# microsoft/DFOL-VQA

Measured on AMD Instinct MI355X. Metric: questions/sec (GQA programs, N=100 objects), higher is better.
Workload: dtype f32

## Files before the change

### dfol_vqa_amd/csrc/dfol_pair_h2.hip

```cpp
#include "dfol_common.h"

#include <stdlib.h>

#include <type_traits>

#ifdef DFOL_PAIR_TRACE
__device__ long long dfol_h2_trace_buf[8 * 8 * 64];
#define TRACE(slot)                                                                                                  \
    do {                                                                                                             \
        if (trace_on && lane == 0) dfol_h2_trace_buf[(trace_blk * 8 + wave) * 64 + (slot)] = clock64();              \
    } while (0)
#else
#define TRACE(slot)
#endif

#ifndef DFOL_H2_PREFETCH
#define DFOL_H2_PREFETCH 1
#endif
#ifndef DFOL_H2_BDEPTH
#define DFOL_H2_BDEPTH 2
#endif
#ifndef DFOL_H2_DMA_ASM
#define DFOL_H2_DMA_ASM 1
#endif
#ifndef DFOL_H2T_SKIP
#define DFOL_H2T_SKIP 0
#endif
#ifndef DFOL_H2_DMA_LATE
#define DFOL_H2_DMA_LATE 0
#endif


namespace {

typedef float floatx4 __attribute__((ext_vector_type(4)));
typedef _Float16 f16x8 __attribute__((ext_vector_type(8)));
typedef _Float16 f16x2 __attribute__((ext_vector_type(2)));
typedef float f32x2 __attribute__((ext_vector_type(2)));
typedef uint32_t u32x4 __attribute__((ext_vector_type(4)));

constexpr float H2_NL2E = -1.44269504088896340736f;
constexpr int H2_CH = 32;
constexpr int H2_ROWS = 320, H2_TILES = 20;
constexpr int H2_PIECES = 2 * H2_ROWS * 4;
constexpr float H2_AMAX = 60000.0f;
constexpr float H2_L2E = 1.44269504088896340736f;
constexpr float H2_LN2 = 0.69314718055994530942f;

__device__ __forceinline__ int h2_swz(int row) { return (4 - ((row >> 2) & 3)) & 3; }

__device__ __forceinline__ void h2_split2(float x0, float x1, uint32_t& h, uint32_t& l) {
    const f32x2 x = {x0, x1};
    const f16x2 hh = __builtin_convertvector(x, f16x2);
    const f32x2 r = x - __builtin_convertvector(hh, f32x2);
    const f16x2 ll = __builtin_convertvector(r, f16x2);
    h = __builtin_bit_cast(uint32_t, hh);
    l = __builtin_bit_cast(uint32_t, ll);
}

__device__ __forceinline__ float h2_elu_neg(float zs) {
    const float p = __builtin_amdgcn_fmed3f(__builtin_amdgcn_exp2f(zs), 0.0f, 1.0f);
    return fmaf(p, H2_L2E, -H2_L2E);
}

__host__ __device__ __forceinline__ constexpr int h2_kperm(int kq, int e) { return 16 * (e >> 2) + 4 * kq + (e & 3); }

template <bool HI>
__device__ __forceinline__ float h2_resid(float x, uint32_t hpair) {
    float r;
    if (HI) asm("v_fma_mix_f32 %0, -%1, 1.0, %2 op_sel:[1,0,0] op_sel_hi:[1,0,0]" : "=v"(r) : "v"(hpair), "v"(x));
    else asm("v_fma_mix_f32 %0, -%1, 1.0, %2 op_sel:[0,0,0] op_sel_hi:[1,0,0]" : "=v"(r) : "v"(hpair), "v"(x));
    return r;
}

__global__ void h2_row_scale_kernel(const float* __restrict__ W2, int64_t ld_w2, int HID2, int HID1, float* __restrict__ tail) {
    const int lane = threadIdx.x & 63, r = blockIdx.x * (blockDim.x >> 6) + (threadIdx.x >> 6);
    if (r >= H2_ROWS) return;
    float m = 0.f;
    if (r < HID2)
        for (int k = lane; k < HID1; k += 64) m = fmaxf(m, fabsf(W2[(int64_t)r * ld_w2 + k] * H2_LN2));
#pragma unroll
    for (int s = 32; s >= 1; s >>= 1) m = fmaxf(m, __shfl_xor(m, s, 64));
    int e = 0;
    if (m > 0.f && m < 3.0e38f) {
        int x;
        (void)frexpf(m, &x);
        e = 14 - x;
        e = e < -100 ? -100 : (e > 100 ? 100 : e);
    }
    if (lane == 0) {
        tail[r] = ldexpf(H2_NL2E, -e);
        reinterpret_cast<int32_t*>(tail)[H2_ROWS + r] = e;
    }
}

__global__ void h2_pack_w2_kernel(const float* __restrict__ W2, int64_t ld_w2, int HID2, int HID1, const float* __restrict__ tail,
                                  u32x4* __restrict__ out) {
    const int idx = blockIdx.x * blockDim.x + threadIdx.x;
    if (idx >= (HID1 / H2_CH) * H2_PIECES) return;
    const int c = idx / H2_PIECES, rem = idx - c * H2_PIECES;
    const int p = rem / (H2_ROWS * 4), rr = rem - p * H2_ROWS * 4, r = rr >> 2, slot = rr & 3;
    const int kq = slot ^ h2_swz(r);
    const int e = reinterpret_cast<const int32_t*>(tail)[H2_ROWS + r];
    uint32_t piece[4];
#pragma unroll
    for (int j = 0; j < 4; ++j) {
        float w0 = 0.f, w1 = 0.f;
        if (r < HID2) {
            w0 = ldexpf(W2[(int64_t)r * ld_w2 + c * H2_CH + h2_kperm(kq, 2 * j)] * H2_LN2, e);
            w1 = ldexpf(W2[(int64_t)r * ld_w2 + c * H2_CH + h2_kperm(kq, 2 * j + 1)] * H2_LN2, e);
        }
        uint32_t h, l;
        h2_split2(w0, w1, h, l);
        piece[j] = p == 0 ? h : l;
    }
    out[idx] = u32x4{piece[0], piece[1], piece[2], piece[3]};
}

struct H2Train {
    float* Z;
    float* pre2;
    int64_t ld_pre2;
    float* geo;
    float* x;
    int64_t ld_x;
    const int64_t* pair_off;
};

template <int NB16, bool TBF16, bool TRAIN = false>
__global__ __launch_bounds__(512) __attribute__((amdgpu_waves_per_eu(2, 2))) void pair_ll32h_kernel(
    const float* UV , int64_t ld_uv, int HID1, const float* __restrict__ pos, int64_t ld_pos,
    const float* __restrict__ Wg, const u32x4* __restrict__ W2h, const float* __restrict__ b2, int HID2,
    const float* __restrict__ E, int64_t ld_e, const float* __restrict__ be, const int32_t* __restrict__ n_obj,
    const int32_t* __restrict__ obj_off, int Q, int tiles_per_image, const int32_t* __restrict__ req_col,
    const int32_t* __restrict__ req_tile, const uint8_t* __restrict__ req_orient, int K, int NS, float dflt,
    void* __restrict__ tiles_v, H2Train tr) {
    constexpr int MT = 2, WAVES = 8;
    constexpr int ROWS = NB16 * 16, T = WAVES * 64, SLOTS = MT * 16 * WAVES;
    static_assert(NB16 > 16 && NB16 <= H2_TILES, "geometry");
    __shared__ __attribute__((aligned(16))) u32x4 Bs[2 * H2_PIECES];
    __shared__ __attribute__((aligned(16))) u32x4 WgA[(256 / H2_CH) * 2 * 64];
    constexpr int STAGE_FLOATS = 8192;
    __shared__ __attribute__((aligned(16))) float stage[STAGE_FLOATS];
    const int q = blockIdx.x / tiles_per_image, tb = blockIdx.x - q * tiles_per_image;
    const int n = n_obj[q], npairs = n * (n - 1);
    if (tb * SLOTS >= npairs) return;
    bool any = TRAIN;
    for (int k = 0; k < K; ++k) any |= req_col[(int64_t)k * Q + q] >= 0;
    if (!any) return;
    const int64_t prow0 = TRAIN ? tr.pair_off[q] : 0;

    const int tid = threadIdx.x, lane = tid & 63, wave = __builtin_amdgcn_readfirstlane(tid >> 6), kh = lane >> 4, r16 = lane & 15;
#ifdef DFOL_PAIR_TRACE
    const int trace_blk = ((int)blockIdx.x - 3000) / 500;
    const bool trace_on = blockIdx.x >= 3000 && (blockIdx.x - 3000) % 500 == 0 && trace_blk < 8;
#endif
    TRACE(0);
    const int nchunk = HID1 / H2_CH, lastc = nchunk - 1;
#pragma unroll
    for (int i = 0; i < H2_PIECES / T; ++i)
        __builtin_amdgcn_global_load_lds(W2h + T * i + tid, (__attribute__((address_space(3))) void*)&Bs[T * i + wave * 64], 16, 0, 0);
    const float* cf = reinterpret_cast<const float*>(W2h + (int64_t)nchunk * H2_PIECES);
    const int first = obj_off[q];
    u32x4 geoB[MT];
    const char* img_uv = reinterpret_cast<const char*>(UV + (int64_t)first * ld_uv);
    uint32_t uoff[MT], voff[MT];
    uint32_t zoff[MT];
#pragma unroll
    for (int m = 0; m < MT; ++m) {
        const int e_slot = tb * SLOTS + wave * (MT * 16) + m * 16 + r16;
        const bool valid = e_slot < npairs;
        zoff[m] = (TRAIN && valid) ? (uint32_t)(e_slot * HID1 + 4 * kh) * 4u : 0xffffffffu;
        const int s = valid ? e_slot / (n - 1) : 0, oo_ = valid ? e_slot - s * (n - 1) : 0, o = oo_ + (oo_ >= s);
        const float* ps = pos + (int64_t)(first + s) * ld_pos;
        const float* po = pos + (int64_t)(first + o) * ld_pos;
        const float x1 = ps[0], y1 = ps[1], w1 = ps[2], h1 = ps[3], x2 = po[0], y2 = po[1], w2 = po[2], h2 = po[3];
        const float dx = x1 + w1 / 2.0f - x2 - w2 / 2.0f, dy = y1 + h1 / 2.0f - y2 - h2 / 2.0f;
        const float dist = sqrtf(dx * dx + dy * dy);
        uint32_t gh01, gl01, gh23, gl23;
        const float ang = asinf(dy / fmaxf(dist, 1e-10f));
        const float sgx = (x2 - x1 > 0.f) ? 1.f : ((x2 - x1 < 0.f) ? -1.f : 0.f), sgy = (y2 - y1 > 0.f) ? 1.f : ((y2 - y1 < 0.f) ? -1.f : 0.f);
        h2_split2(dist, ang, gh01, gl01);
        h2_split2(sgx, sgy, gh23, gl23);
        if (TRAIN && valid && kh == 0) *reinterpret_cast<floatx4*>(tr.geo + (prow0 + e_slot) * 4) = floatx4{dist, ang, sgx, sgy};
        geoB[m] = kh == 0 ? u32x4{gh01, gh23, gl01, gl23} : (kh == 1 ? u32x4{gh01, gh23, 0u, 0u} : u32x4{0u, 0u, 0u, 0u});
        uoff[m] = (uint32_t)(s * (int)ld_uv + 4 * kh) * 4u;
        voff[m] = (uint32_t)(o * (int)ld_uv + HID1 + 4 * kh) * 4u;
    }
    for (int i = tid; i < (HID1 / 16) * 64; i += T) {
        const int kt = i >> 6, ln = i & 63, khh = ln >> 4;
        u32x4 frag = {0u, 0u, 0u, 0u};
        if (khh < 2) {
            const float4 g = *reinterpret_cast<const float4*>(Wg + (kt * 16 + (ln & 15)) * 4);
            uint32_t h01, l01, h23, l23;
            h2_split2(g.x * H2_L2E, g.y * H2_L2E, h01, l01);
            h2_split2(g.z * H2_L2E, g.w * H2_L2E, h23, l23);
            frag = khh == 0 ? u32x4{h01, h23, h01, h23} : u32x4{l01, l23, 0u, 0u};
        }
        WgA[i] = frag;
    }
    constexpr int SR = STAGE_FLOATS / ROWS - 2;
    for (int i = tid; i < ROWS; i += T) {
        stage[i] = H2_NL2E * (i < HID2 ? b2[i] : -1.0e30f);
        stage[ROWS + i] = i < HID2 ? cf[i] : 0.f;
    }
    const int Kc = K < SR ? K : SR;
    for (int k = 0; k < Kc; ++k) {
        const int col = req_col[(int64_t)k * Q + q];
        for (int i = tid; i < ROWS; i += T) stage[ROWS * (2 + k) + i] = (col >= 0 && i < HID2) ? E[(int64_t)col * ld_e + i] : 0.f;
    }

    floatx4 acc[MT][NB16];
#pragma unroll
    for (int m = 0; m < MT; ++m)
#pragma unroll
        for (int i = 0; i < NB16; ++i) acc[m][i] = floatx4{0.f, 0.f, 0.f, 0.f};

    auto dma_chunk = [&](int c, int buf) __attribute__((always_inline)) {
        const int w = wave - 4;
        constexpr int PER_WAVE = H2_PIECES / 4;
        const u32x4* src = W2h + (int64_t)c * H2_PIECES + w * PER_WAVE + lane;
        u32x4* dst = &Bs[buf * H2_PIECES + w * PER_WAVE];
#pragma unroll
        for (int g = 0; g < PER_WAVE / 64; g += 4) {
#if DFOL_H2_DMA_ASM
            const uint32_t d = (uint32_t)(uintptr_t)(__attribute__((address_space(3))) void*)(dst + 64 * g);
            const u32x4* sp = src + 64 * g;
#pragma clang diagnostic push
#pragma clang diagnostic ignored "-Winline-asm"
            const uint32_t m0v = __builtin_amdgcn_readfirstlane(d);
            const int rem = PER_WAVE / 64 - g;
            if (rem >= 4)
                asm volatile("s_mov_b32 m0, %1\n\ts_nop 0\n\tglobal_load_lds_dwordx4 %0, off\n\tglobal_load_lds_dwordx4 %0, off offset:1024\n\t"
                             "global_load_lds_dwordx4 %0, off offset:2048\n\tglobal_load_lds_dwordx4 %0, off offset:3072" ::"v"(sp), "s"(m0v) : "memory", "m0");
            else if (rem == 3)
                asm volatile("s_mov_b32 m0, %1\n\ts_nop 0\n\tglobal_load_lds_dwordx4 %0, off\n\tglobal_load_lds_dwordx4 %0, off offset:1024\n\t"
                             "global_load_lds_dwordx4 %0, off offset:2048" ::"v"(sp), "s"(m0v) : "memory", "m0");
            else if (rem == 2)
                asm volatile("s_mov_b32 m0, %1\n\ts_nop 0\n\tglobal_load_lds_dwordx4 %0, off\n\tglobal_load_lds_dwordx4 %0, off offset:1024" ::"v"(sp), "s"(m0v) : "memory", "m0");
            else
                asm volatile("s_mov_b32 m0, %1\n\ts_nop 0\n\tglobal_load_lds_dwordx4 %0, off" ::"v"(sp), "s"(m0v) : "memory", "m0");
#pragma clang diagnostic pop
#else
            auto d = (__attribute__((address_space(3))) void*)(dst + 64 * g);
            __builtin_amdgcn_global_load_lds(src + 64 * g, d, 16, 0, 0);
            if (g + 1 < PER_WAVE / 64) __builtin_amdgcn_global_load_lds(src + 64 * g, d, 16, 1024, 0);
            if (g + 2 < PER_WAVE / 64) __builtin_amdgcn_global_load_lds(src + 64 * g, d, 16, 2048, 0);
            if (g + 3 < PER_WAVE / 64) __builtin_amdgcn_global_load_lds(src + 64 * g, d, 16, 3072, 0);
#endif
        }
    };
    floatx4 ru[MT][2], rv[MT][2];
    auto load_uv = [&](int c) __attribute__((always_inline)) {
        const char* base = img_uv + (uint32_t)__builtin_amdgcn_readfirstlane(H2_CH * 4 * c);
#pragma unroll
        for (int m = 0; m < MT; ++m)
#pragma unroll
            for (int half = 0; half < 2; ++half) {
                ru[m][half] = *reinterpret_cast<const floatx4*>(base + uoff[m] + 64 * half);
                rv[m][half] = *reinterpret_cast<const floatx4*>(base + voff[m] + 64 * half);
            }
    };
    u32x4 ap[MT][2];
    auto make_a = [&](int c) __attribute__((always_inline)) {
        floatx4 z[MT][2];
#pragma unroll
        for (int t = 0; t < 2; ++t) {
            const f16x8 wa = __builtin_bit_cast(f16x8, WgA[(2 * c + t) * 64 + lane]);
#pragma unroll
            for (int m = 0; m < MT; ++m)
                z[m][t] = __builtin_amdgcn_mfma_f32_16x16x32_f16(wa, __builtin_bit_cast(f16x8, geoB[m]), ru[m][t] + rv[m][t], 0, 0, 0);
        }
#pragma unroll
        for (int m = 0; m < MT; ++m)
#pragma unroll
            for (int t = 0; t < 2; ++t)
#pragma unroll
                for (int jp = 0; jp < 2; ++jp) {
                    const float z0 = z[m][t][2 * jp], z1 = z[m][t][2 * jp + 1];
                    const float a0 = __builtin_amdgcn_fmed3f(z0, h2_elu_neg(z0), H2_AMAX);
                    const float a1 = __builtin_amdgcn_fmed3f(z1, h2_elu_neg(z1), H2_AMAX);
                    const uint32_t hh = __builtin_bit_cast(uint32_t, __builtin_convertvector((f32x2){a0, a1}, f16x2));
                    const uint32_t ll = __builtin_bit_cast(uint32_t, __builtin_convertvector((f32x2){h2_resid<false>(a0, hh), h2_resid<true>(a1, hh)}, f16x2));
                    ap[m][0][2 * t + jp] = hh;
                    ap[m][1][2 * t + jp] = ll;
                    if (TRAIN) z[m][t][2 * jp] = a0 * H2_LN2, z[m][t][2 * jp + 1] = a1 * H2_LN2;
                }
        if (TRAIN && !(DFOL_H2T_SKIP & 1)) {
            char* zimg = reinterpret_cast<char*>(tr.Z + prow0 * HID1) + (uint32_t)__builtin_amdgcn_readfirstlane(H2_CH * 4 * c);
#pragma unroll
            for (int m = 0; m < MT; ++m)
                if (zoff[m] != 0xffffffffu) {
#pragma unroll
                    for (int t = 0; t < 2; ++t) *reinterpret_cast<floatx4*>(zimg + zoff[m] + 64 * t) = z[m][t];
                }
        }
    };
    const int boff = r16 * 4 + (kh ^ h2_swz(r16));
    int bbase = boff;
    auto load_b = [&](int i, f16x8 (&b)[2]) __attribute__((always_inline)) {
#pragma unroll
        for (int p = 0; p < 2; ++p) b[p] = __builtin_bit_cast(f16x8, Bs[bbase + i * 64 + p * H2_ROWS * 4]);
    };
    constexpr int PA3[3] = {1, 0, 0}, PB3[3] = {0, 1, 0};
    auto chunk_mfma = [&]() __attribute__((always_inline)) {
        constexpr int D = DFOL_H2_BDEPTH;
        f16x8 bq[D + 1][2];
#pragma unroll
        for (int d = 0; d < D; ++d) load_b(d, bq[d]);
#pragma unroll
        for (int i = 0; i < NB16; ++i) {
            if (i + D < NB16) load_b(i + D, bq[(i + D) % (D + 1)]);
            __builtin_amdgcn_sched_barrier(0);
#pragma unroll
            for (int m = 0; m < MT; ++m) {
#pragma unroll
                for (int x = 0; x < 3; ++x)
                    acc[m][i] = __builtin_amdgcn_mfma_f32_16x16x32_f16(__builtin_bit_cast(f16x8, ap[m][PA3[x]]), bq[i % (D + 1)][PB3[x]], acc[m][i], 0, 0, 0);
                __builtin_amdgcn_sched_barrier(0);
            }
        }
    };
    __builtin_amdgcn_s_waitcnt(0x0F70);
    __syncthreads();

    auto run_half = [&](auto y_tag) __attribute__((always_inline)) {
        constexpr bool Y = decltype(y_tag)::value;
        TRACE(1);
        if (Y) {
            if (nchunk > 1) dma_chunk(1, 1);
            if (DFOL_H2_PREFETCH) load_uv(0);
            __syncthreads();
        } else if (DFOL_H2_PREFETCH) {
            load_uv(0);
        }
        TRACE(2);
        for (int c = 0; c < nchunk; ++c) {
            if (!DFOL_H2_PREFETCH) load_uv(c);
            if (DFOL_H2_PREFETCH) {
                floatx4 t0 = ru[0][0], t1 = ru[0][1], t2 = ru[1][0], t3 = ru[1][1], t4 = rv[0][0], t5 = rv[0][1], t6 = rv[1][0], t7 = rv[1][1];
                asm volatile("s_waitcnt vmcnt(0)" : "+v"(t0), "+v"(t1), "+v"(t2), "+v"(t3), "+v"(t4), "+v"(t5), "+v"(t6), "+v"(t7));
                ru[0][0] = t0, ru[0][1] = t1, ru[1][0] = t2, ru[1][1] = t3, rv[0][0] = t4, rv[0][1] = t5, rv[1][0] = t6, rv[1][1] = t7;
            }
            TRACE(40 + c);
            if (Y && !DFOL_H2_DMA_LATE && c >= 1 && c < lastc) dma_chunk(c + 1, (c + 1) & 1);
            TRACE(50 + c);
            make_a(c);
#pragma unroll
            for (int m = 0; m < MT; ++m)
#pragma unroll
                for (int p = 0; p < 2; ++p) asm volatile("" : "+v"(ap[m][p]));
            __builtin_amdgcn_sched_barrier(0);
            if (Y && DFOL_H2_DMA_LATE && c >= 1 && c < lastc) dma_chunk(c + 1, (c + 1) & 1);
            TRACE(3 + 4 * c);
            __syncthreads();
            __builtin_amdgcn_sched_barrier(0);
            TRACE(4 + 4 * c);
            bbase = boff + (c & 1) * H2_PIECES;
            if (DFOL_H2_PREFETCH && c < lastc) load_uv(c + 1);
            chunk_mfma();
            if (Y) __builtin_amdgcn_s_waitcnt(0x0F70);
            TRACE(5 + 4 * c);
            if (!Y || c < lastc) __syncthreads();
            TRACE(6 + 4 * c);
        }
    };
    if (wave < 4) run_half(std::false_type());
    else run_half(std::true_type());

    const int64_t tile_sz = (int64_t)NS * NS;
#pragma unroll
    for (int m = 0; m < MT; ++m)
#pragma unroll
        for (int i = 0; i < NB16; ++i) {
            const float bv = stage[i * 16 + r16], cm = stage[ROWS + i * 16 + r16];
            if (TRAIN && !(DFOL_H2T_SKIP & 2)) {
                const int colp = i * 16 + r16;
#pragma unroll
                for (int e = 0; e < 4; ++e) {
                    const int ee = tb * SLOTS + wave * (MT * 16) + m * 16 + 4 * kh + e;
                    if (colp < HID2 && ee < npairs)
                        *reinterpret_cast<float*>(reinterpret_cast<char*>(tr.pre2 + prow0 * tr.ld_pre2) + (uint32_t)(ee * (int)tr.ld_pre2 + colp) * 4u) =
                            -H2_LN2 * fmaf(acc[m][i][e], cm, bv);
                }
            }
#pragma unroll
            for (int e = 0; e < 4; ++e) acc[m][i][e] = __builtin_amdgcn_rcpf(1.0f + __builtin_amdgcn_exp2f(fmaf(acc[m][i][e], cm, bv)));
        }
    for (int k = 0; k < K; ++k) {
        const int col = req_col[(int64_t)k * Q + q];
        if (col < 0) continue;
        float vm[MT];
#pragma unroll
        for (int m = 0; m < MT; ++m) {
            float part[4] = {0.f, 0.f, 0.f, 0.f};
            if (k < Kc) {
                const float* erow = stage + ROWS * (2 + k) + r16;
#pragma unroll
                for (int i = 0; i < NB16; ++i) {
                    const float ev = erow[i * 16];
#pragma unroll
                    for (int e = 0; e < 4; ++e) part[e] = fmaf(acc[m][i][e], ev, part[e]);
                }
            } else {
                const float* erow = E + (int64_t)col * ld_e;
#pragma unroll
                for (int i = 0; i < NB16; ++i) {
                    const float ev = erow[min(i * 16 + r16, HID2 - 1)];
#pragma unroll
                    for (int e = 0; e < 4; ++e) part[e] = fmaf(acc[m][i][e], ev, part[e]);
                }
            }
#pragma unroll
            for (int e = 0; e < 4; ++e) part[e] = dfol_group_sum<16>(part[e]);
            vm[m] = r16 == 0 ? part[0] : (r16 == 1 ? part[1] : (r16 == 2 ? part[2] : part[3]));
        }
        const float shifted = __int_as_float(__builtin_amdgcn_update_dpp(0, __float_as_int(vm[1]), 0x114, 0xF, 0xF, false));
        if (r16 < 8) {
            const int hi = r16 >> 2;
            const float v = hi ? shifted : vm[0];
            const int ee = tb * SLOTS + wave * (MT * 16) + hi * 16 + 4 * kh + (r16 & 3);
            if (ee < npairs) {
                if (TRAIN) {
                    tr.x[(int64_t)k * tr.ld_x + prow0 + ee] = v;
                    continue;
                }
                const int ss = (int)(((float)ee + 0.5f) * __builtin_amdgcn_rcpf((float)(n - 1))), op = ee - ss * (n - 1), oo = op + (op >= ss);
                const float x = v + (be ? be[col] : 0.f);
                const float val = fminf(x, 0.f) - dfol_log(1.0f + dfol_exp(-fabsf(x)));
                const int64_t at = (int64_t)req_tile[(int64_t)k * Q + q] * tile_sz +
                                   ((req_orient && req_orient[(int64_t)k * Q + q]) ? (int64_t)oo * NS + ss : (int64_t)ss * NS + oo);
                if (TBF16) {
                    uint32_t u = __float_as_uint(val);
                    u += 0x7fffu + ((u >> 16) & 1u);
                    reinterpret_cast<uint16_t*>(tiles_v)[at] = (uint16_t)(u >> 16);
                } else {
                    reinterpret_cast<float*>(tiles_v)[at] = val;
                }
            }
        }
    }
    TRACE(60);
}

__global__ __launch_bounds__(512) void h2_uv_range_kernel(const float* __restrict__ UV, int64_t ld_uv, int HID1, const float* __restrict__ pos,
                                                          int64_t ld_pos, const float* __restrict__ Wg, const int32_t* __restrict__ n_obj,
                                                          const int32_t* __restrict__ obj_off, uint32_t* __restrict__ status) {
    __shared__ float4 part[512];
    __shared__ float box[4][8];
    const int q = blockIdx.x, n = n_obj[q], first = obj_off[q], t = threadIdx.x, lane = t & 63, wave = t >> 6;
    if (n < 2) return;
    const int G = (2 * HID1) / 4, R = 512 / G, cg = t % G, rg = t / G;
    float4 m = {-INFINITY, -INFINITY, -INFINITY, -INFINITY};
    bool nan = false;
    const float* base = UV + (int64_t)first * ld_uv + 4 * cg;
    auto take = [&](const float4 a) {
        nan |= (a.x != a.x) | (a.y != a.y) | (a.z != a.z) | (a.w != a.w);
        m.x = fmaxf(m.x, a.x), m.y = fmaxf(m.y, a.y), m.z = fmaxf(m.z, a.z), m.w = fmaxf(m.w, a.w);
    };
    int o = rg;
    for (; o + 3 * R < n; o += 4 * R) {
        const float4 a = *reinterpret_cast<const float4*>(base + (int64_t)o * ld_uv), b = *reinterpret_cast<const float4*>(base + (int64_t)(o + R) * ld_uv);
        const float4 c = *reinterpret_cast<const float4*>(base + (int64_t)(o + 2 * R) * ld_uv), d = *reinterpret_cast<const float4*>(base + (int64_t)(o + 3 * R) * ld_uv);
        take(a), take(b), take(c), take(d);
    }
    for (; o < n; o += R) take(*reinterpret_cast<const float4*>(base + (int64_t)o * ld_uv));
    if (nan) m.x = NAN;
    part[t] = m;
    float lox = INFINITY, hix = -INFINITY, loy = INFINITY, hiy = -INFINITY;
    for (int i = t; i < n; i += 512) {
        const float* p = pos + (int64_t)(first + i) * ld_pos;
        const float cx = p[0] + p[2] / 2.0f, cy = p[1] + p[3] / 2.0f;
        lox = fminf(lox, cx), hix = fmaxf(hix, cx), loy = fminf(loy, cy), hiy = fmaxf(hiy, cy);
    }
#pragma unroll
    for (int s = 32; s >= 1; s >>= 1) {
        lox = fminf(lox, __shfl_xor(lox, s, 64)), hix = fmaxf(hix, __shfl_xor(hix, s, 64));
        loy = fminf(loy, __shfl_xor(loy, s, 64)), hiy = fmaxf(hiy, __shfl_xor(hiy, s, 64));
    }
    if (lane == 0) box[0][wave] = lox, box[1][wave] = hix, box[2][wave] = loy, box[3][wave] = hiy;
    __syncthreads();
    if (t < HID1) {
#pragma unroll
        for (int w = 0; w < 8; ++w) lox = fminf(lox, box[0][w]), hix = fmaxf(hix, box[1][w]), loy = fminf(loy, box[2][w]), hiy = fmaxf(hiy, box[3][w]);
        const float* pf = reinterpret_cast<const float*>(part);
        float mu = -INFINITY, mv = -INFINITY;
        bool bad = false;
        for (int r = 0; r < R; ++r) {
            const float u = pf[(r * G + t / 4) * 4 + (t & 3)], v = pf[(r * G + (HID1 + t) / 4) * 4 + (t & 3)];
            const float ux = pf[(r * G + t / 4) * 4], vx = pf[(r * G + (HID1 + t) / 4) * 4];
            bad |= (ux != ux) | (vx != vx);
            mu = fmaxf(mu, u), mv = fmaxf(mv, v);
        }
        const float dmax = sqrtf((hix - lox) * (hix - lox) + (hiy - loy) * (hiy - loy));
        const float4 g = *reinterpret_cast<const float4*>(Wg + t * 4);
        const float geo = H2_L2E * (fabsf(g.x) * dmax + fabsf(g.y) * 1.57079632679489661923f + fabsf(g.z) + fabsf(g.w));
        const float bound = mu + mv + geo;
        if (bad || !(bound <= H2_AMAX)) atomicOr(status, (uint32_t)DFOL_RANGE_PAIR_SATURATED);
    }
}

}

#ifdef DFOL_PAIR_TRACE
extern "C" int dfol_pair_h2_trace_read(long long* out) { return (int)hipMemcpyFromSymbol(out, HIP_SYMBOL(dfol_h2_trace_buf), sizeof(dfol_h2_trace_buf)); }
#endif

extern "C" int64_t dfol_pair_w2_f16x2_bytes(int32_t HID1) { return (int64_t)(HID1 / H2_CH) * H2_PIECES * 16 + 2 * H2_ROWS * 4; }

extern "C" int dfol_pair_pack_w2_f16x2(const float* W2, int64_t ld_w2, int32_t HID2, int32_t HID1, void* W2_split, void* stream) {
    DFOL_REQUIRE(HID1 > 0 && HID1 <= 256 && HID1 % H2_CH == 0, "pair_pack_w2_f16x2: HID1=%d must be a multiple of %d, <= 256", HID1, H2_CH);
    DFOL_REQUIRE(HID2 > 256 && HID2 <= 320, "pair_pack_w2_f16x2: HID2=%d must be in (256, 320]", HID2);
    DFOL_REQUIRE(W2 && W2_split && ld_w2 >= HID1, "pair_pack_w2_f16x2: null pointer or ld_w2 < HID1");
    DFOL_REQUIRE((uintptr_t)W2_split % 16 == 0, "pair_pack_w2_f16x2: output must be 16-byte aligned");
    const int total = (HID1 / H2_CH) * H2_PIECES;
    float* tail = reinterpret_cast<float*>(reinterpret_cast<u32x4*>(W2_split) + total);
    hipLaunchKernelGGL(h2_row_scale_kernel, dim3(H2_ROWS / 4), dim3(256), 0, (hipStream_t)stream, W2, ld_w2, HID2, HID1, tail);
    hipLaunchKernelGGL(h2_pack_w2_kernel, dim3(dfol_cdiv(total, 256)), dim3(256), 0, (hipStream_t)stream, W2, ld_w2, HID2, HID1, (const float*)tail,
                       (u32x4*)W2_split);
    DFOL_LAUNCH_CHECK("pair_pack_w2_f16x2");
    return 0;
}

extern "C" int dfol_pair_ll_h2_f32(const float* UV, int64_t ld_uv, int32_t HID1, const float* pos, int64_t ld_pos, const float* Wg,
                                   const void* W2_split, const float* b2, int32_t HID2, const float* E, int64_t ld_e,
                                   const float* be, const int32_t* n_obj, const int32_t* obj_off, int32_t Q, int32_t max_n,
                                   const int32_t* req_col, const int32_t* req_tile, const uint8_t* req_orient, int32_t K,
                                   int32_t NS, float default_ll, int32_t tile_dtype, void* tiles_v, void* stream) {
    DFOL_REQUIRE(tile_dtype == DFOL_TILE_F32 || (tile_dtype == DFOL_TILE_BF16 && NS % 8 == 0), "pair_ll_h2: tile_dtype=%d (bf16 tiles need NS %% 8 == 0)", tile_dtype);
    DFOL_REQUIRE(Q >= 0 && K >= 0 && NS > 0 && NS % 4 == 0 && max_n >= 0 && max_n <= NS, "pair_ll_h2: bad sizes Q=%d K=%d NS=%d max_n=%d", Q, K, NS, max_n);
    DFOL_REQUIRE(HID1 > 0 && HID1 <= 256 && HID1 % H2_CH == 0 && ld_uv % 4 == 0, "pair_ll_h2: HID1=%d must be a multiple of %d, <= 256, UV rows 16-byte aligned", HID1, H2_CH);
    DFOL_REQUIRE(HID2 > 256 && HID2 <= 320, "pair_ll_h2: HID2=%d must be in (256, 320]", HID2);
    if (Q == 0 || K == 0 || max_n < 2) return 0;
    DFOL_REQUIRE(UV && pos && Wg && W2_split && b2 && E && n_obj && obj_off && req_col && req_tile && tiles_v, "pair_ll_h2: null pointer");
    DFOL_REQUIRE(((uintptr_t)UV % 16 == 0) && ((uintptr_t)W2_split % 16 == 0) && ((uintptr_t)Wg % 16 == 0), "pair_ll_h2: operands must be 16-byte aligned");
    hipStream_t st = (hipStream_t)stream;
    const int tpi = dfol_cdiv((int64_t)max_n * (max_n - 1), 256);
    DFOL_REQUIRE((int64_t)Q * tpi < ((int64_t)1 << 31), "pair_ll_h2: too many tiles");
    DFOL_REQUIRE((int64_t)max_n * ld_uv * 4 < ((int64_t)1 << 31), "pair_ll_h2: an image's U / V rows must span less than 2 GB");
    const dim3 grid((unsigned)Q * tpi);
    if (uint32_t* status = dfol_range_status_ptr())
        hipLaunchKernelGGL(h2_uv_range_kernel, dim3((unsigned)Q), dim3(512), 0, st, UV, ld_uv, HID1, pos, ld_pos, Wg, n_obj, obj_off, status);
    const H2Train none = {nullptr, nullptr, 0, nullptr, nullptr, 0, nullptr};
#define DFOL_PAIR32H(NBV, BF)                                                                                                       \
    hipLaunchKernelGGL((pair_ll32h_kernel<NBV, BF>), grid, dim3(512), 0, st, UV, ld_uv, HID1, pos, ld_pos, Wg, (const u32x4*)W2_split, b2, HID2, \
                       E, ld_e, be, n_obj, obj_off, Q, tpi, req_col, req_tile, req_orient, K, NS, default_ll, tiles_v, none)
    if (HID2 <= 272) { if (tile_dtype == DFOL_TILE_BF16) DFOL_PAIR32H(17, true); else DFOL_PAIR32H(17, false); }
    else if (HID2 <= 288) { if (tile_dtype == DFOL_TILE_BF16) DFOL_PAIR32H(18, true); else DFOL_PAIR32H(18, false); }
    else if (HID2 <= 304) { if (tile_dtype == DFOL_TILE_BF16) DFOL_PAIR32H(19, true); else DFOL_PAIR32H(19, false); }
    else { if (tile_dtype == DFOL_TILE_BF16) DFOL_PAIR32H(20, true); else DFOL_PAIR32H(20, false); }
#undef DFOL_PAIR32H
    DFOL_LAUNCH_CHECK("pair_ll_h2");
    return 0;
}


extern "C" int dfol_pair_train_fwd_h2_f32(const float* UV, int64_t ld_uv, int32_t HID1, const float* pos, int64_t ld_pos, const float* Wg,
                                          const void* W2_split, const float* b2, int32_t HID2, const float* E, int64_t ld_e, const int32_t* n_obj,
                                          const int32_t* obj_off, const int64_t* pair_off, int32_t Q, int32_t max_n, const int32_t* req_row, int32_t K,
                                          float* Z, float* pre2, int64_t ld_pre2, float* geo, float* x, int64_t ld_x, void* stream) {
    DFOL_REQUIRE(Q >= 0 && K >= 0 && max_n >= 0, "pair_train_fwd_h2: bad sizes Q=%d K=%d max_n=%d", Q, K, max_n);
    DFOL_REQUIRE(HID1 > 0 && HID1 <= 256 && HID1 % H2_CH == 0 && ld_uv % 4 == 0, "pair_train_fwd_h2: HID1=%d must be a multiple of %d, <= 256, UV rows 16-byte aligned", HID1, H2_CH);
    DFOL_REQUIRE(HID2 > 256 && HID2 <= 320 && ld_pre2 >= HID2, "pair_train_fwd_h2: HID2=%d must be in (256, 320], ld_pre2 >= HID2", HID2);
    if (Q == 0 || max_n < 2) return 0;
    DFOL_REQUIRE(UV && pos && Wg && W2_split && b2 && n_obj && obj_off && pair_off && Z && pre2 && geo && (K == 0 || (E && req_row && x)), "pair_train_fwd_h2: null pointer");
    DFOL_REQUIRE(((uintptr_t)UV % 16 == 0) && ((uintptr_t)W2_split % 16 == 0) && ((uintptr_t)Wg % 16 == 0) && ((uintptr_t)Z % 16 == 0) && ((uintptr_t)geo % 16 == 0),
                 "pair_train_fwd_h2: operands must be 16-byte aligned");
    hipStream_t st = (hipStream_t)stream;
    const int tpi = dfol_cdiv((int64_t)max_n * (max_n - 1), 256);
    DFOL_REQUIRE((int64_t)Q * tpi < ((int64_t)1 << 31), "pair_train_fwd_h2: too many tiles");
    DFOL_REQUIRE((int64_t)max_n * ld_uv * 4 < ((int64_t)1 << 31) && (int64_t)max_n * (max_n - 1) * HID1 * 4 < ((int64_t)1 << 32) - 1,
                 "pair_train_fwd_h2: an image's rows must span less than 2 GB (U | V) / 4 GB (Z)");
    if (uint32_t* status = dfol_range_status_ptr())
        hipLaunchKernelGGL(h2_uv_range_kernel, dim3((unsigned)Q), dim3(512), 0, st, UV, ld_uv, HID1, pos, ld_pos, Wg, n_obj, obj_off, status);
    const H2Train tr = {Z, pre2, ld_pre2, geo, x, ld_x, pair_off};
    const dim3 grid((unsigned)Q * tpi);
#define DFOL_PAIR32T(NBV)                                                                                                                    \
    hipLaunchKernelGGL((pair_ll32h_kernel<NBV, false, true>), grid, dim3(512), 0, st, UV, ld_uv, HID1, pos, ld_pos, Wg, (const u32x4*)W2_split, b2, HID2, \
                       E, ld_e, (const float*)nullptr, n_obj, obj_off, Q, tpi, req_row, (const int32_t*)nullptr, (const uint8_t*)nullptr, K, 4, 0.f,      \
                       (void*)nullptr, tr)
    if (HID2 <= 272) DFOL_PAIR32T(17);
    else if (HID2 <= 288) DFOL_PAIR32T(18);
    else if (HID2 <= 304) DFOL_PAIR32T(19);
    else DFOL_PAIR32T(20);
#undef DFOL_PAIR32T
    DFOL_LAUNCH_CHECK("pair_train_fwd_h2");
    return 0;
}
```

Before: 180,800.

## Make pair kernel persistent over several tiles per workgroup

Each workgroup of the inference pair kernel now loops over a contiguous run of wg_tiles pair tiles (default 4, overridable via DFOL_PAIR_TILES) instead of one, so the grid shrinks accordingly. The first W2 chunk DMA is issued only once per workgroup, which amortises launch, setup and weight-loading overhead across tiles. The cost is fewer workgroups and so less parallelism and tail balancing, plus extra register pressure from wrapping the body in a loop. Training keeps one tile per workgroup.

```diff
diff --git a/dfol_vqa_amd/csrc/dfol_pair_h2.hip b/dfol_vqa_amd/csrc/dfol_pair_h2.hip
--- a/dfol_vqa_amd/csrc/dfol_pair_h2.hip
+++ b/dfol_vqa_amd/csrc/dfol_pair_h2.hip
@@ -129,10 +129,10 @@
 
 template <int NB16, bool TBF16, bool TRAIN = false>
 __global__ __launch_bounds__(512) __attribute__((amdgpu_waves_per_eu(2, 2))) void pair_ll32h_kernel(
-    const float* UV , int64_t ld_uv, int HID1, const float* __restrict__ pos, int64_t ld_pos,
-    const float* __restrict__ Wg, const u32x4* __restrict__ W2h, const float* __restrict__ b2, int HID2,
-    const float* __restrict__ E, int64_t ld_e, const float* __restrict__ be, const int32_t* __restrict__ n_obj,
-    const int32_t* __restrict__ obj_off, int Q, int tiles_per_image, const int32_t* __restrict__ req_col,
+    const float* UV_ , int64_t ld_uv_, int HID1, const float* __restrict__ pos_, int64_t ld_pos_,
+    const float* __restrict__ Wg_, const u32x4* __restrict__ W2h_, const float* __restrict__ b2_, int HID2,
+    const float* __restrict__ E_, int64_t ld_e, const float* __restrict__ be, const int32_t* __restrict__ n_obj,
+    const int32_t* __restrict__ obj_off, int Q, int tiles_per_image, int wg_tiles, const int32_t* __restrict__ req_col,
     const int32_t* __restrict__ req_tile, const uint8_t* __restrict__ req_orient, int K, int NS, float dflt,
     void* __restrict__ tiles_v, H2Train tr) {
     constexpr int MT = 2, WAVES = 8;
@@ -142,305 +142,350 @@
     __shared__ __attribute__((aligned(16))) u32x4 WgA[(256 / H2_CH) * 2 * 64];
     constexpr int STAGE_FLOATS = 8192;
     __shared__ __attribute__((aligned(16))) float stage[STAGE_FLOATS];
-    const int q = blockIdx.x / tiles_per_image, tb = blockIdx.x - q * tiles_per_image;
-    const int n = n_obj[q], npairs = n * (n - 1);
-    if (tb * SLOTS >= npairs) return;
-    bool any = TRAIN;
-    for (int k = 0; k < K; ++k) any |= req_col[(int64_t)k * Q + q] >= 0;
-    if (!any) return;
-    const int64_t prow0 = TRAIN ? tr.pair_off[q] : 0;
-
-    const int tid = threadIdx.x, lane = tid & 63, wave = __builtin_amdgcn_readfirstlane(tid >> 6), kh = lane >> 4, r16 = lane & 15;
+
+    const int wave = __builtin_amdgcn_readfirstlane((int)threadIdx.x >> 6);
 #ifdef DFOL_PAIR_TRACE
-    const int trace_blk = ((int)blockIdx.x - 3000) / 500;
-    const bool trace_on = blockIdx.x >= 3000 && (blockIdx.x - 3000) % 500 == 0 && trace_blk < 8;
-#endif
-    TRACE(0);
+    const int trace_b0 = 3000 / wg_tiles, trace_step = 500 / wg_tiles > 0 ? 500 / wg_tiles : 1;
+    const int trace_blk = ((int)blockIdx.x - trace_b0) / trace_step;
+    const bool trace_on = (int)blockIdx.x >= trace_b0 && ((int)blockIdx.x - trace_b0) % trace_step == 0 && trace_blk < 8;
+#endif
     const int nchunk = HID1 / H2_CH, lastc = nchunk - 1;
-#pragma unroll
-    for (int i = 0; i < H2_PIECES / T; ++i)
-        __builtin_amdgcn_global_load_lds(W2h + T * i + tid, (__attribute__((address_space(3))) void*)&Bs[T * i + wave * 64], 16, 0, 0);
-    const float* cf = reinterpret_cast<const float*>(W2h + (int64_t)nchunk * H2_PIECES);
-    const int first = obj_off[q];
-    u32x4 geoB[MT];
-    const char* img_uv = reinterpret_cast<const char*>(UV + (int64_t)first * ld_uv);
-    uint32_t uoff[MT], voff[MT];
-    uint32_t zoff[MT];
-#pragma unroll
-    for (int m = 0; m < MT; ++m) {
-        const int e_slot = tb * SLOTS + wave * (MT * 16) + m * 16 + r16;
-        const bool valid = e_slot < npairs;
-        zoff[m] = (TRAIN && valid) ? (uint32_t)(e_slot * HID1 + 4 * kh) * 4u : 0xffffffffu;
-        const int s = valid ? e_slot / (n - 1) : 0, oo_ = valid ? e_slot - s * (n - 1) : 0, o = oo_ + (oo_ >= s);
-        const float* ps = pos + (int64_t)(first + s) * ld_pos;
-        const float* po = pos + (int64_t)(first + o) * ld_pos;
-        const float x1 = ps[0], y1 = ps[1], w1 = ps[2], h1 = ps[3], x2 = po[0], y2 = po[1], w2 = po[2], h2 = po[3];
-        const float dx = x1 + w1 / 2.0f - x2 - w2 / 2.0f, dy = y1 + h1 / 2.0f - y2 - h2 / 2.0f;
-        const float dist = sqrtf(dx * dx + dy * dy);
-        uint32_t gh01, gl01, gh23, gl23;
-        const float ang = asinf(dy / fmaxf(dist, 1e-10f));
-        const float sgx = (x2 - x1 > 0.f) ? 1.f : ((x2 - x1 < 0.f) ? -1.f : 0.f), sgy = (y2 - y1 > 0.f) ? 1.f : ((y2 - y1 < 0.f) ? -1.f : 0.f);
-        h2_split2(dist, ang, gh01, gl01);
-        h2_split2(sgx, sgy, gh23, gl23);
-        if (TRAIN && valid && kh == 0) *reinterpret_cast<floatx4*>(tr.geo + (prow0 + e_slot) * 4) = floatx4{dist, ang, sgx, sgy};
-        geoB[m] = kh == 0 ? u32x4{gh01, gh23, gl01, gl23} : (kh == 1 ? u32x4{gh01, gh23, 0u, 0u} : u32x4{0u, 0u, 0u, 0u});
-        uoff[m] = (uint32_t)(s * (int)ld_uv + 4 * kh) * 4u;
-        voff[m] = (uint32_t)(o * (int)ld_uv + HID1 + 4 * kh) * 4u;
-    }
-    for (int i = tid; i < (HID1 / 16) * 64; i += T) {
-        const int kt = i >> 6, ln = i & 63, khh = ln >> 4;
-        u32x4 frag = {0u, 0u, 0u, 0u};
-        if (khh < 2) {
-            const float4 g = *reinterpret_cast<const float4*>(Wg + (kt * 16 + (ln & 15)) * 4);
-            uint32_t h01, l01, h23, l23;
-            h2_split2(g.x * H2_L2E, g.y * H2_L2E, h01, l01);
-            h2_split2(g.z * H2_L2E, g.w * H2_L2E, h23, l23);
-            frag = khh == 0 ? u32x4{h01, h23, h01, h23} : u32x4{l01, l23, 0u, 0u};
-        }
-        WgA[i] = frag;
-    }
-    constexpr int SR = STAGE_FLOATS / ROWS - 2;
-    for (int i = tid; i < ROWS; i += T) {
-        stage[i] = H2_NL2E * (i < HID2 ? b2[i] : -1.0e30f);
-        stage[ROWS + i] = i < HID2 ? cf[i] : 0.f;
-    }
-    const int Kc = K < SR ? K : SR;
-    for (int k = 0; k < Kc; ++k) {
-        const int col = req_col[(int64_t)k * Q + q];
-        for (int i = tid; i < ROWS; i += T) stage[ROWS * (2 + k) + i] = (col >= 0 && i < HID2) ? E[(int64_t)col * ld_e + i] : 0.f;
-    }
-
-    floatx4 acc[MT][NB16];
-#pragma unroll
-    for (int m = 0; m < MT; ++m)
-#pragma unroll
-        for (int i = 0; i < NB16; ++i) acc[m][i] = floatx4{0.f, 0.f, 0.f, 0.f};
-
-    auto dma_chunk = [&](int c, int buf) __attribute__((always_inline)) {
-        const int w = wave - 4;
-        constexpr int PER_WAVE = H2_PIECES / 4;
-        const u32x4* src = W2h + (int64_t)c * H2_PIECES + w * PER_WAVE + lane;
-        u32x4* dst = &Bs[buf * H2_PIECES + w * PER_WAVE];
-#pragma unroll
-        for (int g = 0; g < PER_WAVE / 64; g += 4) {
+    const int tile_end = (int)min((int64_t)blockIdx.x * wg_tiles + wg_tiles, (int64_t)Q * tiles_per_image);
+    auto dma_chunk0_all = [&](const u32x4* W2h) __attribute__((always_inline)) {
+        int tid = threadIdx.x;
+        asm volatile("" : "+v"(tid));
+#pragma unroll
+        for (int i = 0; i < H2_PIECES / T; ++i)
+            __builtin_amdgcn_global_load_lds(W2h + T * i + tid, (__attribute__((address_space(3))) void*)&Bs[T * i + wave * 64], 16, 0, 0);
+    };
+    bool started = false;
+    bool b0 = false;
+    int stage_q = -1;
+    for (int tile = (int)blockIdx.x * wg_tiles; tile < tile_end; tile = TRAIN ? tile_end : tile + 1) {
+        const int q = tile / tiles_per_image, tb = tile - q * tiles_per_image;
+        const int n = n_obj[q], npairs = n * (n - 1);
+        if (tb * SLOTS >= npairs) continue;
+        bool any = TRAIN;
+        for (int k = 0; k < K; ++k) any |= req_col[(int64_t)k * Q + q] >= 0;
+        if (!any) continue;
+        const int64_t prow0 = TRAIN ? tr.pair_off[q] : 0;
+        const u32x4* W2h = W2h_;
+        const float *Wg = Wg_, *b2 = b2_, *E = E_, *UV = UV_, *pos = pos_;
+        int64_t ld_uv = ld_uv_, ld_pos = ld_pos_;
+        asm volatile("" : "+s"(W2h), "+s"(Wg), "+s"(b2), "+s"(E));
+        asm volatile("" : "+s"(UV), "+s"(pos), "+s"(ld_uv), "+s"(ld_pos));
+        int tid = threadIdx.x;
+        asm volatile("" : "+v"(tid));
+        const int lane = tid & 63, kh = lane >> 4, r16 = lane & 15;
+        const float* cf = reinterpret_cast<const float*>(W2h + (int64_t)nchunk * H2_PIECES);
+
+        TRACE(0);
+        if (!started) dma_chunk0_all(W2h);
+        const int first = obj_off[q];
+        u32x4 geoB[MT];
+        const char* img_uv = reinterpret_cast<const char*>(UV + (int64_t)first * ld_uv);
+        uint32_t uoff[MT], voff[MT];
+        uint32_t zoff[MT];
+        auto slot_geometry = [&]() __attribute__((always_inline)) {
+#pragma unroll
+            for (int m = 0; m < MT; ++m) {
+                const int e_slot = tb * SLOTS + wave * (MT * 16) + m * 16 + r16;
+                const bool valid = e_slot < npairs;
+                zoff[m] = (TRAIN && valid) ? (uint32_t)(e_slot * HID1 + 4 * kh) * 4u : 0xffffffffu;
+                const int s = valid ? e_slot / (n - 1) : 0, oo_ = valid ? e_slot - s * (n - 1) : 0, o = oo_ + (oo_ >= s);
+                const float* ps = pos + (int64_t)(first + s) * ld_pos;
+                const float* po = pos + (int64_t)(first + o) * ld_pos;
+                const float x1 = ps[0], y1 = ps[1], w1 = ps[2], h1 = ps[3], x2 = po[0], y2 = po[1], w2 = po[2], h2 = po[3];
+                const float dx = x1 + w1 / 2.0f - x2 - w2 / 2.0f, dy = y1 + h1 / 2.0f - y2 - h2 / 2.0f;
+                const float dist = sqrtf(dx * dx + dy * dy);
+                uint32_t gh01, gl01, gh23, gl23;
+                const float ang = asinf(dy / fmaxf(dist, 1e-10f));
+                const float sgx = (x2 - x1 > 0.f) ? 1.f : ((x2 - x1 < 0.f) ? -1.f : 0.f), sgy = (y2 - y1 > 0.f) ? 1.f : ((y2 - y1 < 0.f) ? -1.f : 0.f);
+                h2_split2(dist, ang, gh01, gl01);
+                h2_split2(sgx, sgy, gh23, gl23);
+                if (TRAIN && valid && kh == 0) *reinterpret_cast<floatx4*>(tr.geo + (prow0 + e_slot) * 4) = floatx4{dist, ang, sgx, sgy};
+                geoB[m] = kh == 0 ? u32x4{gh01, gh23, gl01, gl23} : (kh == 1 ? u32x4{gh01, gh23, 0u, 0u} : u32x4{0u, 0u, 0u, 0u});
+                uoff[m] = (uint32_t)(s * (int)ld_uv + 4 * kh) * 4u;
+                voff[m] = (uint32_t)(o * (int)ld_uv + HID1 + 4 * kh) * 4u;
+            }
+        };
+        constexpr int SR = STAGE_FLOATS / ROWS - 2;
+        const int Kc = K < SR ? K : SR;
+        floatx4 acc[MT][NB16];
+#pragma unroll
+        for (int m = 0; m < MT; ++m)
+#pragma unroll
+            for (int i = 0; i < NB16; ++i) acc[m][i] = floatx4{0.f, 0.f, 0.f, 0.f};
+
+        auto dma_chunk = [&](int c, int buf, int w, int ln) __attribute__((always_inline)) {
+            constexpr int PER_WAVE = H2_PIECES / 4;
+            const u32x4* src = W2h + (int64_t)c * H2_PIECES + w * PER_WAVE + ln;
+            u32x4* dst = &Bs[buf * H2_PIECES + w * PER_WAVE];
+#pragma unroll
+            for (int g = 0; g < PER_WAVE / 64; g += 4) {
 #if DFOL_H2_DMA_ASM
-            const uint32_t d = (uint32_t)(uintptr_t)(__attribute__((address_space(3))) void*)(dst + 64 * g);
-            const u32x4* sp = src + 64 * g;
+                const uint32_t d = (uint32_t)(uintptr_t)(__attribute__((address_space(3))) void*)(dst + 64 * g);
+                const u32x4* sp = src + 64 * g;
 #pragma clang diagnostic push
 #pragma clang diagnostic ignored "-Winline-asm"
-            const uint32_t m0v = __builtin_amdgcn_readfirstlane(d);
-            const int rem = PER_WAVE / 64 - g;
-            if (rem >= 4)
-                asm volatile("s_mov_b32 m0, %1\n\ts_nop 0\n\tglobal_load_lds_dwordx4 %0, off\n\tglobal_load_lds_dwordx4 %0, off offset:1024\n\t"
-                             "global_load_lds_dwordx4 %0, off offset:2048\n\tglobal_load_lds_dwordx4 %0, off offset:3072" ::"v"(sp), "s"(m0v) : "memory", "m0");
-            else if (rem == 3)
-                asm volatile("s_mov_b32 m0, %1\n\ts_nop 0\n\tglobal_load_lds_dwordx4 %0, off\n\tglobal_load_lds_dwordx4 %0, off offset:1024\n\t"
-                             "global_load_lds_dwordx4 %0, off offset:2048" ::"v"(sp), "s"(m0v) : "memory", "m0");
-            else if (rem == 2)
-                asm volatile("s_mov_b32 m0, %1\n\ts_nop 0\n\tglobal_load_lds_dwordx4 %0, off\n\tglobal_load_lds_dwordx4 %0, off offset:1024" ::"v"(sp), "s"(m0v) : "memory", "m0");
-            else
-                asm volatile("s_mov_b32 m0, %1\n\ts_nop 0\n\tglobal_load_lds_dwordx4 %0, off" ::"v"(sp), "s"(m0v) : "memory", "m0");
+                const uint32_t m0v = __builtin_amdgcn_readfirstlane(d);
+                const int rem = PER_WAVE / 64 - g;
+                if (rem >= 4)
+                    asm volatile("s_mov_b32 m0, %1\n\ts_nop 0\n\tglobal_load_lds_dwordx4 %0, off\n\tglobal_load_lds_dwordx4 %0, off offset:1024\n\t"
+                                 "global_load_lds_dwordx4 %0, off offset:2048\n\tglobal_load_lds_dwordx4 %0, off offset:3072" ::"v"(sp), "s"(m0v) : "memory", "m0");
+                else if (rem == 3)
+                    asm volatile("s_mov_b32 m0, %1\n\ts_nop 0\n\tglobal_load_lds_dwordx4 %0, off\n\tglobal_load_lds_dwordx4 %0, off offset:1024\n\t"
+                                 "global_load_lds_dwordx4 %0, off offset:2048" ::"v"(sp), "s"(m0v) : "memory", "m0");
+                else if (rem == 2)
+                    asm volatile("s_mov_b32 m0, %1\n\ts_nop 0\n\tglobal_load_lds_dwordx4 %0, off\n\tglobal_load_lds_dwordx4 %0, off offset:1024" ::"v"(sp), "s"(m0v) : "memory", "m0");
+                else
+                    asm volatile("s_mov_b32 m0, %1\n\ts_nop 0\n\tglobal_load_lds_dwordx4 %0, off" ::"v"(sp), "s"(m0v) : "memory", "m0");
 #pragma clang diagnostic pop
 #else
-            auto d = (__attribute__((address_space(3))) void*)(dst + 64 * g);
-            __builtin_amdgcn_global_load_lds(src + 64 * g, d, 16, 0, 0);
-            if (g + 1 < PER_WAVE / 64) __builtin_amdgcn_global_load_lds(src + 64 * g, d, 16, 1024, 0);
-            if (g + 2 < PER_WAVE / 64) __builtin_amdgcn_global_load_lds(src + 64 * g, d, 16, 2048, 0);
-            if (g + 3 < PER_WAVE / 64) __builtin_amdgcn_global_load_lds(src + 64 * g, d, 16, 3072, 0);
-#endif
+                auto d = (__attribute__((address_space(3))) void*)(dst + 64 * g);
+                __builtin_amdgcn_global_load_lds(src + 64 * g, d, 16, 0, 0);
+                if (g + 1 < PER_WAVE / 64) __builtin_amdgcn_global_load_lds(src + 64 * g, d, 16, 1024, 0);
+                if (g + 2 < PER_WAVE / 64) __builtin_amdgcn_global_load_lds(src + 64 * g, d, 16, 2048, 0);
+                if (g + 3 < PER_WAVE / 64) __builtin_amdgcn_global_load_lds(src + 64 * g, d, 16, 3072, 0);
+#endif
+            }
+        };
+        floatx4 ru[MT][2], rv[MT][2];
+        auto load_uv = [&](int c) __attribute__((always_inline)) {
+            const char* base = img_uv + (uint32_t)__builtin_amdgcn_readfirstlane(H2_CH * 4 * c);
+#pragma unroll
+            for (int m = 0; m < MT; ++m)
+#pragma unroll
+                for (int half = 0; half < 2; ++half) {
+                    ru[m][half] = *reinterpret_cast<const floatx4*>(base + uoff[m] + 64 * half);
+                    rv[m][half] = *reinterpret_cast<const floatx4*>(base + voff[m] + 64 * half);
+                }
+        };
+        u32x4 ap[MT][2];
+        auto make_a = [&](int c) __attribute__((always_inline)) {
+            floatx4 z[MT][2];
+#pragma unroll
+            for (int t = 0; t < 2; ++t) {
+                const f16x8 wa = __builtin_bit_cast(f16x8, WgA[(2 * c + t) * 64 + lane]);
+#pragma unroll
+                for (int m = 0; m < MT; ++m)
+                    z[m][t] = __builtin_amdgcn_mfma_f32_16x16x32_f16(wa, __builtin_bit_cast(f16x8, geoB[m]), ru[m][t] + rv[m][t], 0, 0, 0);
+            }
+#pragma unroll
+            for (int m = 0; m < MT; ++m)
+#pragma unroll
+                for (int t = 0; t < 2; ++t)
+#pragma unroll
+                    for (int jp = 0; jp < 2; ++jp) {
+                        const float z0 = z[m][t][2 * jp], z1 = z[m][t][2 * jp + 1];
+                        const float a0 = __builtin_amdgcn_fmed3f(z0, h2_elu_neg(z0), H2_AMAX);
+                        const float a1 = __builtin_amdgcn_fmed3f(z1, h2_elu_neg(z1), H2_AMAX);
+                        const uint32_t hh = __builtin_bit_cast(uint32_t, __builtin_convertvector((f32x2){a0, a1}, f16x2));
+                        const uint32_t ll = __builtin_bit_cast(uint32_t, __builtin_convertvector((f32x2){h2_resid<false>(a0, hh), h2_resid<true>(a1, hh)}, f16x2));
+                        ap[m][0][2 * t + jp] = hh;
+                        ap[m][1][2 * t + jp] = ll;
+                        if (TRAIN) z[m][t][2 * jp] = a0 * H2_LN2, z[m][t][2 * jp + 1] = a1 * H2_LN2;
+                    }
+            if (TRAIN && !(DFOL_H2T_SKIP & 1)) {
+                char* zimg = reinterpret_cast<char*>(tr.Z + prow0 * HID1) + (uint32_t)__builtin_amdgcn_readfirstlane(H2_CH * 4 * c);
+#pragma unroll
+                for (int m = 0; m < MT; ++m)
+                    if (zoff[m] != 0xffffffffu) {
+#pragma unroll
+                        for (int t = 0; t < 2; ++t) *reinterpret_cast<floatx4*>(zimg + zoff[m] + 64 * t) = z[m][t];
+                    }
+            }
+        };
+        const int boff = r16 * 4 + (kh ^ h2_swz(r16));
+        int bbase = boff;
+        auto load_b = [&](int i, f16x8 (&b)[2]) __attribute__((always_inline)) {
+#pragma unroll
+            for (int p = 0; p < 2; ++p) b[p] = __builtin_bit_cast(f16x8, Bs[bbase + i * 64 + p * H2_ROWS * 4]);
+        };
+        constexpr int PA3[3] = {1, 0, 0}, PB3[3] = {0, 1, 0};
+        auto chunk_mfma = [&]() __attribute__((always_inline)) {
+            constexpr int D = DFOL_H2_BDEPTH;
+            f16x8 bq[D + 1][2];
+#pragma unroll
+            for (int d = 0; d < D; ++d) load_b(d, bq[d]);
+#pragma unroll
+            for (int i = 0; i < NB16; ++i) {
+                if (i + D < NB16) load_b(i + D, bq[(i + D) % (D + 1)]);
+                __builtin_amdgcn_sched_barrier(0);
+#pragma unroll
+                for (int m = 0; m < MT; ++m) {
+#pragma unroll
+                    for (int x = 0; x < 3; ++x)
+                        acc[m][i] = __builtin_amdgcn_mfma_f32_16x16x32_f16(__builtin_bit_cast(f16x8, ap[m][PA3[x]]), bq[i % (D + 1)][PB3[x]], acc[m][i], 0, 0, 0);
+                    __builtin_amdgcn_sched_barrier(0);
+                }
+            }
+        };
+        slot_geometry();
+        if (started) {
+            __syncthreads();
+            if (!b0) dma_chunk0_all(W2h);
+        } else {
+            int tid = threadIdx.x;
+            asm volatile("" : "+v"(tid));
+            for (int i = tid; i < (HID1 / 16) * 64; i += T) {
+                const int kt = i >> 6, ln = i & 63, khh = ln >> 4;
+                u32x4 frag = {0u, 0u, 0u, 0u};
+                if (khh < 2) {
+                    const float4 g = *reinterpret_cast<const float4*>(Wg + (kt * 16 + (ln & 15)) * 4);
+                    uint32_t h01, l01, h23, l23;
+                    h2_split2(g.x * H2_L2E, g.y * H2_L2E, h01, l01);
+                    h2_split2(g.z * H2_L2E, g.w * H2_L2E, h23, l23);
+                    frag = khh == 0 ? u32x4{h01, h23, h01, h23} : u32x4{l01, l23, 0u, 0u};
+                }
+                WgA[i] = frag;
+            }
         }
-    };
-    floatx4 ru[MT][2], rv[MT][2];
-    auto load_uv = [&](int c) __attribute__((always_inline)) {
-        const char* base = img_uv + (uint32_t)__builtin_amdgcn_readfirstlane(H2_CH * 4 * c);
+        if (q != stage_q) {
+            int tid = threadIdx.x;
+            asm volatile("" : "+v"(tid));
+            for (int i = tid; i < ROWS; i += T) {
+                stage[i] = H2_NL2E * (i < HID2 ? b2[i] : -1.0e30f);
+                stage[ROWS + i] = i < HID2 ? cf[i] : 0.f;
+            }
+            for (int k = 0; k < Kc; ++k) {
+                const int col = req_col[(int64_t)k * Q + q];
+                for (int i = tid; i < ROWS; i += T) stage[ROWS * (2 + k) + i] = (col >= 0 && i < HID2) ? E[(int64_t)col * ld_e + i] : 0.f;
+            }
+        }
+        __builtin_amdgcn_s_waitcnt(0x0F70);
+        __syncthreads();
+
+        const bool pf = (lastc & 1) && tile + 1 < tile_end;
+        auto run_half = [&](auto y_tag) __attribute__((always_inline)) {
+            constexpr bool Y = decltype(y_tag)::value;
+            TRACE(1);
+            if (Y) {
+                if (nchunk > 1) dma_chunk(1, 1, wave - 4, lane);
+                if (DFOL_H2_PREFETCH) load_uv(0);
+                __syncthreads();
+            } else if (DFOL_H2_PREFETCH) {
+                load_uv(0);
+            }
+            TRACE(2);
+            for (int c = 0; c < nchunk; ++c) {
+                if (!DFOL_H2_PREFETCH) load_uv(c);
+                if (DFOL_H2_PREFETCH) {
+                    floatx4 t0 = ru[0][0], t1 = ru[0][1], t2 = ru[1][0], t3 = ru[1][1], t4 = rv[0][0], t5 = rv[0][1], t6 = rv[1][0], t7 = rv[1][1];
+                    asm volatile("s_waitcnt vmcnt(0)" : "+v"(t0), "+v"(t1), "+v"(t2), "+v"(t3), "+v"(t4), "+v"(t5), "+v"(t6), "+v"(t7));
+                    ru[0][0] = t0, ru[0][1] = t1, ru[1][0] = t2, ru[1][1] = t3, rv[0][0] = t4, rv[0][1] = t5, rv[1][0] = t6, rv[1][1] = t7;
+                }
+                TRACE(40 + c);
+                if (Y && !DFOL_H2_DMA_LATE && c >= 1 && c < lastc) dma_chunk(c + 1, (c + 1) & 1, wave - 4, lane);
+                TRACE(50 + c);
+                make_a(c);
+#pragma unroll
+                for (int m = 0; m < MT; ++m)
+#pragma unroll
+                    for (int p = 0; p < 2; ++p) asm volatile("" : "+v"(ap[m][p]));
+                __builtin_amdgcn_sched_barrier(0);
+                if (Y && DFOL_H2_DMA_LATE && c >= 1 && c < lastc) dma_chunk(c + 1, (c + 1) & 1, wave - 4, lane);
+                TRACE(3 + 4 * c);
+                __syncthreads();
+                __builtin_amdgcn_sched_barrier(0);
+                TRACE(4 + 4 * c);
+                bbase = boff + (c & 1) * H2_PIECES;
+                if (DFOL_H2_PREFETCH && c < lastc) load_uv(c + 1);
+                chunk_mfma();
+                if (Y) __builtin_amdgcn_s_waitcnt(0x0F70);
+                TRACE(5 + 4 * c);
+                if (!Y || c < lastc) __syncthreads();
+                TRACE(6 + 4 * c);
+            }
+            if (!Y && pf) {
+                int ln = lane;
+                asm volatile("" : "+v"(ln));
+                dma_chunk(0, 0, wave, ln);
+            }
+        };
+        if (wave < 4) run_half(std::false_type());
+        else run_half(std::true_type());
+
+        const int64_t tile_sz = (int64_t)NS * NS;
 #pragma unroll
         for (int m = 0; m < MT; ++m)
 #pragma unroll
-            for (int half = 0; half < 2; ++half) {
-                ru[m][half] = *reinterpret_cast<const floatx4*>(base + uoff[m] + 64 * half);
-                rv[m][half] = *reinterpret_cast<const floatx4*>(base + voff[m] + 64 * half);
-            }
-    };
-    u32x4 ap[MT][2];
-    auto make_a = [&](int c) __attribute__((always_inline)) {
-        floatx4 z[MT][2];
-#pragma unroll
-        for (int t = 0; t < 2; ++t) {
-            const f16x8 wa = __builtin_bit_cast(f16x8, WgA[(2 * c + t) * 64 + lane]);
-#pragma unroll
-            for (int m = 0; m < MT; ++m)
-                z[m][t] = __builtin_amdgcn_mfma_f32_16x16x32_f16(wa, __builtin_bit_cast(f16x8, geoB[m]), ru[m][t] + rv[m][t], 0, 0, 0);
+            for (int i = 0; i < NB16; ++i) {
+                const float bv = stage[i * 16 + r16], cm = stage[ROWS + i * 16 + r16];
+                if (TRAIN && !(DFOL_H2T_SKIP & 2)) {
+                    const int colp = i * 16 + r16;
+#pragma unroll
+                    for (int e = 0; e < 4; ++e) {
+                        const int ee = tb * SLOTS + wave * (MT * 16) + m * 16 + 4 * kh + e;
+                        if (colp < HID2 && ee < npairs)
+                            *reinterpret_cast<float*>(reinterpret_cast<char*>(tr.pre2 + prow0 * tr.ld_pre2) + (uint32_t)(ee * (int)tr.ld_pre2 + colp) * 4u) =
+                                -H2_LN2 * fmaf(acc[m][i][e], cm, bv);
+                    }
+                }
+#pragma unroll
+                for (int e = 0; e < 4; ++e) acc[m][i][e] = __builtin_amdgcn_rcpf(1.0f + __builtin_amdgcn_exp2f(fmaf(acc[m][i][e], cm, bv)));
+            }
+        for (int k = 0; k < K; ++k) {
+            const int col = req_col[(int64_t)k * Q + q];
+            if (col < 0) continue;
+            float vm[MT];
+#pragma unroll
+            for (int m = 0; m < MT; ++m) {
+                float part[4] = {0.f, 0.f, 0.f, 0.f};
+                if (k < Kc) {
+                    const float* erow = stage + ROWS * (2 + k) + r16;
+#pragma unroll
+                    for (int i = 0; i < NB16; ++i) {
+                        const float ev = erow[i * 16];
+#pragma unroll
+                        for (int e = 0; e < 4; ++e) part[e] = fmaf(acc[m][i][e], ev, part[e]);
+                    }
+                } else {
+                    const float* erow = E + (int64_t)col * ld_e;
+                    int c16 = r16;
+                    asm volatile("" : "+v"(c16));
+#pragma unroll
+                    for (int i = 0; i < NB16; ++i) {
+                        const float ev = erow[min(i * 16 + c16, HID2 - 1)];
+#pragma unroll
+                        for (int e = 0; e < 4; ++e) part[e] = fmaf(acc[m][i][e], ev, part[e]);
+                    }
+                }
+#pragma unroll
+                for (int e = 0; e < 4; ++e) part[e] = dfol_group_sum<16>(part[e]);
+                vm[m] = r16 == 0 ? part[0] : (r16 == 1 ? part[1] : (r16 == 2 ? part[2] : part[3]));
+            }
+            const float shifted = __int_as_float(__builtin_amdgcn_update_dpp(0, __float_as_int(vm[1]), 0x114, 0xF, 0xF, false));
+            if (r16 < 8) {
+                const int hi = r16 >> 2;
+                const float v = hi ? shifted : vm[0];
+                const int ee = tb * SLOTS + wave * (MT * 16) + hi * 16 + 4 * kh + (r16 & 3);
+                if (ee < npairs) {
+                    if (TRAIN) {
+                        tr.x[(int64_t)k * tr.ld_x + prow0 + ee] = v;
+                        continue;
+                    }
+                    const int ss = (int)(((float)ee + 0.5f) * __builtin_amdgcn_rcpf((float)(n - 1))), op = ee - ss * (n - 1), oo = op + (op >= ss);
+                    const float x = v + (be ? be[col] : 0.f);
+                    const float val = fminf(x, 0.f) - dfol_log(1.0f + dfol_exp(-fabsf(x)));
+                    const int64_t at = (int64_t)req_tile[(int64_t)k * Q + q] * tile_sz +
+                                       ((req_orient && req_orient[(int64_t)k * Q + q]) ? (int64_t)oo * NS + ss : (int64_t)ss * NS + oo);
+                    if (TBF16) {
+                        uint32_t u = __float_as_uint(val);
+                        u += 0x7fffu + ((u >> 16) & 1u);
+                        reinterpret_cast<uint16_t*>(tiles_v)[at] = (uint16_t)(u >> 16);
+                    } else {
+                        reinterpret_cast<float*>(tiles_v)[at] = val;
+                    }
+                }
+            }
         }
-#pragma unroll
-        for (int m = 0; m < MT; ++m)
-#pragma unroll
-            for (int t = 0; t < 2; ++t)
-#pragma unroll
-                for (int jp = 0; jp < 2; ++jp) {
-                    const float z0 = z[m][t][2 * jp], z1 = z[m][t][2 * jp + 1];
-                    const float a0 = __builtin_amdgcn_fmed3f(z0, h2_elu_neg(z0), H2_AMAX);
-                    const float a1 = __builtin_amdgcn_fmed3f(z1, h2_elu_neg(z1), H2_AMAX);
-                    const uint32_t hh = __builtin_bit_cast(uint32_t, __builtin_convertvector((f32x2){a0, a1}, f16x2));
-                    const uint32_t ll = __builtin_bit_cast(uint32_t, __builtin_convertvector((f32x2){h2_resid<false>(a0, hh), h2_resid<true>(a1, hh)}, f16x2));
-                    ap[m][0][2 * t + jp] = hh;
-                    ap[m][1][2 * t + jp] = ll;
-                    if (TRAIN) z[m][t][2 * jp] = a0 * H2_LN2, z[m][t][2 * jp + 1] = a1 * H2_LN2;
-                }
-        if (TRAIN && !(DFOL_H2T_SKIP & 1)) {
-            char* zimg = reinterpret_cast<char*>(tr.Z + prow0 * HID1) + (uint32_t)__builtin_amdgcn_readfirstlane(H2_CH * 4 * c);
-#pragma unroll
-            for (int m = 0; m < MT; ++m)
-                if (zoff[m] != 0xffffffffu) {
-#pragma unroll
-                    for (int t = 0; t < 2; ++t) *reinterpret_cast<floatx4*>(zimg + zoff[m] + 64 * t) = z[m][t];
-                }
-        }
-    };
-    const int boff = r16 * 4 + (kh ^ h2_swz(r16));
-    int bbase = boff;
-    auto load_b = [&](int i, f16x8 (&b)[2]) __attribute__((always_inline)) {
-#pragma unroll
-        for (int p = 0; p < 2; ++p) b[p] = __builtin_bit_cast(f16x8, Bs[bbase + i * 64 + p * H2_ROWS * 4]);
-    };
-    constexpr int PA3[3] = {1, 0, 0}, PB3[3] = {0, 1, 0};
-    auto chunk_mfma = [&]() __attribute__((always_inline)) {
-        constexpr int D = DFOL_H2_BDEPTH;
-        f16x8 bq[D + 1][2];
-#pragma unroll
-        for (int d = 0; d < D; ++d) load_b(d, bq[d]);
-#pragma unroll
-        for (int i = 0; i < NB16; ++i) {
-            if (i + D < NB16) load_b(i + D, bq[(i + D) % (D + 1)]);
-            __builtin_amdgcn_sched_barrier(0);
-#pragma unroll
-            for (int m = 0; m < MT; ++m) {
-#pragma unroll
-                for (int x = 0; x < 3; ++x)
-                    acc[m][i] = __builtin_amdgcn_mfma_f32_16x16x32_f16(__builtin_bit_cast(f16x8, ap[m][PA3[x]]), bq[i % (D + 1)][PB3[x]], acc[m][i], 0, 0, 0);
-                __builtin_amdgcn_sched_barrier(0);
-            }
-        }
-    };
+        TRACE(60);
+        started = true;
+        stage_q = q;
+        b0 = pf;
+    }
     __builtin_amdgcn_s_waitcnt(0x0F70);
-    __syncthreads();
-
-    auto run_half = [&](auto y_tag) __attribute__((always_inline)) {
-        constexpr bool Y = decltype(y_tag)::value;
-        TRACE(1);
-        if (Y) {
-            if (nchunk > 1) dma_chunk(1, 1);
-            if (DFOL_H2_PREFETCH) load_uv(0);
-            __syncthreads();
-        } else if (DFOL_H2_PREFETCH) {
-            load_uv(0);
-        }
-        TRACE(2);
-        for (int c = 0; c < nchunk; ++c) {
-            if (!DFOL_H2_PREFETCH) load_uv(c);
-            if (DFOL_H2_PREFETCH) {
-                floatx4 t0 = ru[0][0], t1 = ru[0][1], t2 = ru[1][0], t3 = ru[1][1], t4 = rv[0][0], t5 = rv[0][1], t6 = rv[1][0], t7 = rv[1][1];
-                asm volatile("s_waitcnt vmcnt(0)" : "+v"(t0), "+v"(t1), "+v"(t2), "+v"(t3), "+v"(t4), "+v"(t5), "+v"(t6), "+v"(t7));
-                ru[0][0] = t0, ru[0][1] = t1, ru[1][0] = t2, ru[1][1] = t3, rv[0][0] = t4, rv[0][1] = t5, rv[1][0] = t6, rv[1][1] = t7;
-            }
-            TRACE(40 + c);
-            if (Y && !DFOL_H2_DMA_LATE && c >= 1 && c < lastc) dma_chunk(c + 1, (c + 1) & 1);
-            TRACE(50 + c);
-            make_a(c);
-#pragma unroll
-            for (int m = 0; m < MT; ++m)
-#pragma unroll
-                for (int p = 0; p < 2; ++p) asm volatile("" : "+v"(ap[m][p]));
-            __builtin_amdgcn_sched_barrier(0);
-            if (Y && DFOL_H2_DMA_LATE && c >= 1 && c < lastc) dma_chunk(c + 1, (c + 1) & 1);
-            TRACE(3 + 4 * c);
-            __syncthreads();
-            __builtin_amdgcn_sched_barrier(0);
-            TRACE(4 + 4 * c);
-            bbase = boff + (c & 1) * H2_PIECES;
-            if (DFOL_H2_PREFETCH && c < lastc) load_uv(c + 1);
-            chunk_mfma();
-            if (Y) __builtin_amdgcn_s_waitcnt(0x0F70);
-            TRACE(5 + 4 * c);
-            if (!Y || c < lastc) __syncthreads();
-            TRACE(6 + 4 * c);
-        }
-    };
-    if (wave < 4) run_half(std::false_type());
-    else run_half(std::true_type());
-
-    const int64_t tile_sz = (int64_t)NS * NS;
-#pragma unroll
-    for (int m = 0; m < MT; ++m)
-#pragma unroll
-        for (int i = 0; i < NB16; ++i) {
-            const float bv = stage[i * 16 + r16], cm = stage[ROWS + i * 16 + r16];
-            if (TRAIN && !(DFOL_H2T_SKIP & 2)) {
-                const int colp = i * 16 + r16;
-#pragma unroll
-                for (int e = 0; e < 4; ++e) {
-                    const int ee = tb * SLOTS + wave * (MT * 16) + m * 16 + 4 * kh + e;
-                    if (colp < HID2 && ee < npairs)
-                        *reinterpret_cast<float*>(reinterpret_cast<char*>(tr.pre2 + prow0 * tr.ld_pre2) + (uint32_t)(ee * (int)tr.ld_pre2 + colp) * 4u) =
-                            -H2_LN2 * fmaf(acc[m][i][e], cm, bv);
-                }
-            }
-#pragma unroll
-            for (int e = 0; e < 4; ++e) acc[m][i][e] = __builtin_amdgcn_rcpf(1.0f + __builtin_amdgcn_exp2f(fmaf(acc[m][i][e], cm, bv)));
-        }
-    for (int k = 0; k < K; ++k) {
-        const int col = req_col[(int64_t)k * Q + q];
-        if (col < 0) continue;
-        float vm[MT];
-#pragma unroll
-        for (int m = 0; m < MT; ++m) {
-            float part[4] = {0.f, 0.f, 0.f, 0.f};
-            if (k < Kc) {
-                const float* erow = stage + ROWS * (2 + k) + r16;
-#pragma unroll
-                for (int i = 0; i < NB16; ++i) {
-                    const float ev = erow[i * 16];
-#pragma unroll
-                    for (int e = 0; e < 4; ++e) part[e] = fmaf(acc[m][i][e], ev, part[e]);
-                }
-            } else {
-                const float* erow = E + (int64_t)col * ld_e;
-#pragma unroll
-                for (int i = 0; i < NB16; ++i) {
-                    const float ev = erow[min(i * 16 + r16, HID2 - 1)];
-#pragma unroll
-                    for (int e = 0; e < 4; ++e) part[e] = fmaf(acc[m][i][e], ev, part[e]);
-                }
-            }
-#pragma unroll
-            for (int e = 0; e < 4; ++e) part[e] = dfol_group_sum<16>(part[e]);
-            vm[m] = r16 == 0 ? part[0] : (r16 == 1 ? part[1] : (r16 == 2 ? part[2] : part[3]));
-        }
-        const float shifted = __int_as_float(__builtin_amdgcn_update_dpp(0, __float_as_int(vm[1]), 0x114, 0xF, 0xF, false));
-        if (r16 < 8) {
-            const int hi = r16 >> 2;
-            const float v = hi ? shifted : vm[0];
-            const int ee = tb * SLOTS + wave * (MT * 16) + hi * 16 + 4 * kh + (r16 & 3);
-            if (ee < npairs) {
-                if (TRAIN) {
-                    tr.x[(int64_t)k * tr.ld_x + prow0 + ee] = v;
-                    continue;
-                }
-                const int ss = (int)(((float)ee + 0.5f) * __builtin_amdgcn_rcpf((float)(n - 1))), op = ee - ss * (n - 1), oo = op + (op >= ss);
-                const float x = v + (be ? be[col] : 0.f);
-                const float val = fminf(x, 0.f) - dfol_log(1.0f + dfol_exp(-fabsf(x)));
-                const int64_t at = (int64_t)req_tile[(int64_t)k * Q + q] * tile_sz +
-                                   ((req_orient && req_orient[(int64_t)k * Q + q]) ? (int64_t)oo * NS + ss : (int64_t)ss * NS + oo);
-                if (TBF16) {
-                    uint32_t u = __float_as_uint(val);
-                    u += 0x7fffu + ((u >> 16) & 1u);
-                    reinterpret_cast<uint16_t*>(tiles_v)[at] = (uint16_t)(u >> 16);
-                } else {
-                    reinterpret_cast<float*>(tiles_v)[at] = val;
-                }
-            }
-        }
-    }
-    TRACE(60);
 }
 
 __global__ __launch_bounds__(512) void h2_uv_range_kernel(const float* __restrict__ UV, int64_t ld_uv, int HID1, const float* __restrict__ pos,
@@ -506,6 +551,15 @@
 extern "C" int dfol_pair_h2_trace_read(long long* out) { return (int)hipMemcpyFromSymbol(out, HIP_SYMBOL(dfol_h2_trace_buf), sizeof(dfol_h2_trace_buf)); }
 #endif
 
+#ifndef DFOL_H2_WG_TILES
+#define DFOL_H2_WG_TILES 4
+#endif
+static int h2_wg_tiles() {
+    const char* e = getenv("DFOL_PAIR_TILES");
+    const int t = e ? atoi(e) : DFOL_H2_WG_TILES;
+    return t < 1 ? 1 : (t > 64 ? 64 : t);
+}
+
 extern "C" int64_t dfol_pair_w2_f16x2_bytes(int32_t HID1) { return (int64_t)(HID1 / H2_CH) * H2_PIECES * 16 + 2 * H2_ROWS * 4; }
 
 extern "C" int dfol_pair_pack_w2_f16x2(const float* W2, int64_t ld_w2, int32_t HID2, int32_t HID1, void* W2_split, void* stream) {
@@ -538,13 +592,14 @@
     const int tpi = dfol_cdiv((int64_t)max_n * (max_n - 1), 256);
     DFOL_REQUIRE((int64_t)Q * tpi < ((int64_t)1 << 31), "pair_ll_h2: too many tiles");
     DFOL_REQUIRE((int64_t)max_n * ld_uv * 4 < ((int64_t)1 << 31), "pair_ll_h2: an image's U / V rows must span less than 2 GB");
-    const dim3 grid((unsigned)Q * tpi);
+    const int wgt = h2_wg_tiles();
+    const dim3 grid((unsigned)dfol_cdiv((int64_t)Q * tpi, wgt));
     if (uint32_t* status = dfol_range_status_ptr())
         hipLaunchKernelGGL(h2_uv_range_kernel, dim3((unsigned)Q), dim3(512), 0, st, UV, ld_uv, HID1, pos, ld_pos, Wg, n_obj, obj_off, status);
     const H2Train none = {nullptr, nullptr, 0, nullptr, nullptr, 0, nullptr};
 #define DFOL_PAIR32H(NBV, BF)                                                                                                       \
     hipLaunchKernelGGL((pair_ll32h_kernel<NBV, BF>), grid, dim3(512), 0, st, UV, ld_uv, HID1, pos, ld_pos, Wg, (const u32x4*)W2_split, b2, HID2, \
-                       E, ld_e, be, n_obj, obj_off, Q, tpi, req_col, req_tile, req_orient, K, NS, default_ll, tiles_v, none)
+                       E, ld_e, be, n_obj, obj_off, Q, tpi, wgt, req_col, req_tile, req_orient, K, NS, default_ll, tiles_v, none)
     if (HID2 <= 272) { if (tile_dtype == DFOL_TILE_BF16) DFOL_PAIR32H(17, true); else DFOL_PAIR32H(17, false); }
     else if (HID2 <= 288) { if (tile_dtype == DFOL_TILE_BF16) DFOL_PAIR32H(18, true); else DFOL_PAIR32H(18, false); }
     else if (HID2 <= 304) { if (tile_dtype == DFOL_TILE_BF16) DFOL_PAIR32H(19, true); else DFOL_PAIR32H(19, false); }
@@ -574,10 +629,11 @@
     if (uint32_t* status = dfol_range_status_ptr())
         hipLaunchKernelGGL(h2_uv_range_kernel, dim3((unsigned)Q), dim3(512), 0, st, UV, ld_uv, HID1, pos, ld_pos, Wg, n_obj, obj_off, status);
     const H2Train tr = {Z, pre2, ld_pre2, geo, x, ld_x, pair_off};
+    const int wgt = 1;
     const dim3 grid((unsigned)Q * tpi);
 #define DFOL_PAIR32T(NBV)                                                                                                                    \
     hipLaunchKernelGGL((pair_ll32h_kernel<NBV, false, true>), grid, dim3(512), 0, st, UV, ld_uv, HID1, pos, ld_pos, Wg, (const u32x4*)W2_split, b2, HID2, \
-                       E, ld_e, (const float*)nullptr, n_obj, obj_off, Q, tpi, req_row, (const int32_t*)nullptr, (const uint8_t*)nullptr, K, 4, 0.f,      \
+                       E, ld_e, (const float*)nullptr, n_obj, obj_off, Q, tpi, wgt, req_row, (const int32_t*)nullptr, (const uint8_t*)nullptr, K, 4, 0.f,      \
                        (void*)nullptr, tr)
     if (HID2 <= 272) DFOL_PAIR32T(17);
     else if (HID2 <= 288) DFOL_PAIR32T(18);
```

After: 186,400, median of 6. 3.1% higher.
